# NoemieJaquier/GaBOtorch

Hardware: AMD Instinct MI355X
Metric: SPD affine-invariant kernel-matrix build, pairs/sec (N=4096,d=10) (higher is better)
Workload: dtype f64

## Files before the change

gabotorch_amd/csrc/gabo_mirror.hpp:

```cpp
#pragma once
#include "gabo_device.hpp"

namespace gabo {

template <int TAG>
__global__ __launch_bounds__(256) void mirror_upper_kernel(double* __restrict__ out, int64_t n, int tiles) {
    __shared__ double tile[32][33];
    const int64_t b = blockIdx.y;
    int64_t t = blockIdx.x;
    int ti = 0;
    while (t >= tiles - ti) { t -= tiles - ti; ++ti; }
    int tj = ti + (int)t;
    double* o = out + b * n * n;
    const int tx = threadIdx.x & 31, ty = threadIdx.x >> 5;
    for (int r = ty; r < 32; r += 8) {
        int64_t i = (int64_t)ti * 32 + r, j = (int64_t)tj * 32 + tx;
        tile[r][tx] = (i < n && j < n) ? o[i * n + j] : 0.0;
    }
    __syncthreads();
    for (int r = ty; r < 32; r += 8) {
        int64_t j = (int64_t)tj * 32 + r, i = (int64_t)ti * 32 + tx;
        if (i < n && j < n && i < j) o[j * n + i] = tile[tx][r];
    }
}

__host__ __device__ inline int64_t sym_chunks_of(int64_t cg, int cols, int rows, int64_t row_chunks) {
    int64_t cnt = ((cg + 1) * (int64_t)cols + rows - 1) / rows;
    return cnt < row_chunks ? cnt : row_chunks;
}

__host__ __device__ inline void lower_tile_of(int64_t t, int64_t& bi, int64_t& bj) {
    int64_t r = (int64_t)((__builtin_sqrt(8.0 * (double)t + 1.0) - 1.0) * 0.5);
    while (r * (r + 1) / 2 > t) --r;
    while ((r + 1) * (r + 2) / 2 <= t) ++r;
    bi = r;
    bj = t - r * (r + 1) / 2;
}

}
```

gabotorch_amd/csrc/spd_pairwise_body.hpp:

```cpp
#pragma once
#include "gabo_device.hpp"
#include "spd_eig.hpp"
#include "spd_prep.hpp"
#include "gabo_mirror.hpp"
#include "spd_generic.hpp"
#include "gabo_log_tab.hpp"
#include "gabo_exp_tab256.hpp"
#include "gabo_acosh2_table.hpp"
#include "../../include/gabo_hip.h"

#ifndef GABO_PAIR_WAVES
#define GABO_PAIR_WAVES 2
#else
#define GABO_PAIR_WAVES_FORCED 1
#endif

namespace gabo {

typedef const double __attribute__((address_space(1)))* spd_gcol_ptr;

struct SpdGcolBuffer {
    __amdgpu_buffer_rsrc_t rsrc;
    int voff;
    int stride_bytes;
// ... 31 lines not shown
    constexpr SpdWGroups<D, (GABO_PAIR_WLIM < D ? D : GABO_PAIR_WLIM)> kG{};
    double gq[D][D];
    double wq[2][D][D];
    double c[D];
    auto issue_g = [&](auto ss) {
        constexpr int col = D - 1 - decltype(ss)::value;
        static_for<D - col>([&](auto kk) { gq[col][decltype(kk)::value] = Gj[tri(col + decltype(kk)::value, col)]; });
    };
    auto issue_w = [&](auto gg) {
        constexpr int g = decltype(gg)::value, col = kG.col[g], r0 = kG.r0[g], r1 = kG.r1[g];
        typedef const double __attribute__((address_space(4)))* wrow_ptr;
        wrow_ptr Wg = (wrow_ptr)W;
        asm volatile("" : "+s"(Wg));
        static_for<r1 - r0>([&](auto rr) {
            constexpr int r = r0 + decltype(rr)::value;
            static_for<r - col + 1>([&](auto kk) { wq[g & 1][r][col + decltype(kk)::value] = Wg[tri(r, col + decltype(kk)::value)]; });
        });
    };
    static_for<(AHEAD < D ? AHEAD : D)>(issue_g);
    issue_w(std::integral_constant<int, 0>{});
    static_for<kG.n>([&](auto gg) {
        constexpr int g = decltype(gg)::value, col = kG.col[g], r0 = kG.r0[g], r1 = kG.r1[g];
        if constexpr (r0 == col && D - 1 - col + AHEAD < D) issue_g(std::integral_constant<int, D - 1 - col + AHEAD>{});
        __builtin_amdgcn_sched_barrier(0);
        __builtin_amdgcn_s_waitcnt(0xc07f);
        __builtin_amdgcn_sched_barrier(0);
        if constexpr (g + 1 < kG.n) issue_w(std::integral_constant<int, g + 1>{});
        static_for<r1 - r0>([&](auto rr) {
            constexpr int r = r0 + decltype(rr)::value;
            double acc = wq[g & 1][r][col] * gq[col][0];
            static_for<r - col>([&](auto kk) {
                constexpr int k = col + 1 + decltype(kk)::value;
                acc = __builtin_fma(wq[g & 1][r][k], gq[col][k - col], acc);
            });
            c[r - col] = acc;
        });
        if constexpr (r1 == D) {
            __builtin_amdgcn_sched_barrier(0);
            static_for<D - col>([&](auto rr) {
                constexpr int r = col + decltype(rr)::value;
                static_for<r - col + 1>([&](auto qq) {
                    constexpr int q = col + decltype(qq)::value;
                    m[tri(r, q)] = col == q ? c[r - col] * c[q - col] : __builtin_fma(c[r - col], c[q - col], m[tri(r, q)]);
                });
            });
        }
    });
    __builtin_amdgcn_sched_barrier(0);
}

__constant__ double kLogTabRegs[8] = {1.41421356237309504880, 1.0 / 7.0, -1.0 / 6.0, 0.2, -0.25, 1.0 / 3.0, 6.93147180369123816490e-01,
                                      1.90821492927058770002e-10};
__device__ __forceinline__ LogTabRegs log_tab_regs_scalar() {
    typedef const double __attribute__((address_space(4)))* const_ptr;
    const_ptr p = (const_ptr)kLogTabRegs;
    asm volatile("" : "+s"(p));
    LogTabRegs t;
    t.sqrt2 = p[0], t.c7 = p[1], t.c6 = p[2], t.c5 = p[3], t.c4 = p[4], t.c3 = p[5], t.ln2_hi = p[6], t.ln2_lo = p[7];
    return t;
}

template <int D, int ORIENT = kQlOrientPerLane, int CTL = kQlCtlPlain, int AHEAD = 0, class GCOL>
__device__ __forceinline__ double ai_sumsq(const double* __restrict__ W, const GCOL& Gj, const double* __restrict__ ltab, const double eps2 = 0.0) {
    constexpr int T = tri_size(D);
    constexpr bool kDescending = ORIENT == kQlOrientLast;
    double m[T];
    if constexpr (AHEAD > 0) {
        static_assert(kDescending, "the staged congruence takes the columns from the last to the first");
        ai_congruence_staged<D, AHEAD>(W, Gj, m);
    } else
    static_for<D>([&](auto cc) {
        constexpr int col = kDescending ? D - 1 - decltype(cc)::value : decltype(cc)::value;
        double g[D - col], c[D - col];
        static_for<D - col>([&](auto kk) { g[decltype(kk)::value] = Gj[tri(col + decltype(kk)::value, col)]; });
        static_for<D - col>([&](auto rr) {
            constexpr int r = col + decltype(rr)::value;
            double acc = W[tri(r, col)] * g[0];
            static_for<r - col>([&](auto kk) {
                constexpr int k = col + 1 + decltype(kk)::value;
                acc = __builtin_fma(W[tri(r, k)], g[k - col], acc);
            });
            c[r - col] = acc;
        });
        static_for<D - col>([&](auto rr) {
            constexpr int r = col + decltype(rr)::value;
            static_for<r - col + 1>([&](auto qq) {
                constexpr int q = col + decltype(qq)::value;
                m[tri(r, q)] = (kDescending ? col == q : col == 0) ? c[r - col] * c[q - col] : __builtin_fma(c[r - col], c[q - col], m[tri(r, q)]);
            });
        });
    });
    double dg[D], e2[D];
    tridiagonalize<D, ORIENT>(m, dg, e2);
    tridiag_eigenvalues<D, ORIENT, CTL>(dg, e2, eps2);
    double s = 0.0;
    const LogTabRegs lr = AHEAD > 0 ? log_tab_regs_scalar() : LogTabRegs::load();
    static_for<D>([&](auto kk) { double lg = log_tab(dg[decltype(kk)::value], lr, ltab); s = __builtin_fma(lg, lg, s); });
    return s;
}

struct Spd2Col {
    double g00, g10, g11, lg;
};
__device__ __forceinline__ double ai_sumsq2(const double* __restrict__ W, const Spd2Col& g, double lw, const LogTabRegs& lr,
                                            const double* __restrict__ ltab, double tiny) {
    const double c00 = W[0] * g.g00, c11 = W[2] * g.g11;
    const double c10 = __builtin_fma(W[1], g.g00, W[2] * g.g10);
    const double m00 = c00 * c00, m10d = (c10 + c10) * c00, m11 = __builtin_fma(c10, c10, c11 * c11);
    const double tr = m00 + m11, df = m00 - m11;
    const double root = sqrt_nz(__builtin_fma(df, df, __builtin_fma(m10d, m10d, tiny)));
    const double l1 = log_tab(0.5 * (tr + root), lr, ltab);
    const double l2 = __builtin_fma(2.0, lw + g.lg, -l1);
    return __builtin_fma(l1, l1, l2 * l2);
}

__device__ __forceinline__ double finish(double dist, double beta, int mode) {
    if (mode == GABO_OUT_DISTANCE) return dist;
    if (mode == GABO_OUT_LAPLACE) return exp(-(dist * beta));
    return exp(-((dist * dist) * beta));
}

#ifndef GABO_PAIR_TWO_WAVE_MAX_DIM
#define GABO_PAIR_TWO_WAVE_MAX_DIM 14
#endif
#ifndef GABO_QL_EPS2_GAUSS
#define GABO_QL_EPS2_GAUSS 1e-14
#endif
constexpr bool spd_pair_gauss_only_instantiated(int d) { return d > 2 && d != 12; }
#ifndef GABO_PAIR_ORIENT
constexpr int spd_pair_gauss_only_orientation(int d) { return d == 14 ? kQlOrientCol0 : kQlOrientLast; }
#else
constexpr int spd_pair_gauss_only_orientation(int d) { return GABO_PAIR_ORIENT; }
#endif
#ifndef GABO_PAIR_SWEEPCTL
constexpr int spd_pair_gauss_only_sweepctl(int d) { return d == 20 ? kQlCtlPlain : (kQlCtlDenormalZero | kQlCtlHwSqrt | kQlCtlStageThreshold); }
#else
constexpr int spd_pair_gauss_only_sweepctl(int d) { return GABO_PAIR_SWEEPCTL; }
#endif
#ifndef GABO_PAIR_WAVES_FORCED
constexpr int spd_pair_gauss_only_waves(int d) { return d > GABO_PAIR_TWO_WAVE_MAX_DIM ? 1 : (d == 10 ? 3 : GABO_PAIR_WAVES); }
#else
constexpr int spd_pair_gauss_only_waves(int d) { return d > GABO_PAIR_TWO_WAVE_MAX_DIM ? 1 : GABO_PAIR_WAVES; }
#endif
#ifndef GABO_PAIR_AHEAD
constexpr int spd_pair_gauss_only_ahead(int d) { return d == 10 && spd_pair_gauss_only_waves(d) == 3 ? 2 : 0; }
#else
constexpr int spd_pair_gauss_only_ahead(int d) { return d == 10 ? GABO_PAIR_AHEAD : 0; }
#endif
template <int D, bool GAUSS_ONLY, bool BUFFER_ONLY>
__global__ __launch_bounds__(256, (GAUSS_ONLY ? spd_pair_gauss_only_waves(D) : (D > GABO_PAIR_TWO_WAVE_MAX_DIM ? 1 : GABO_PAIR_WAVES))) void spd_ai_pairwise_kernel(const double* __restrict__ Winv, const double* __restrict__ G,
                                                              double* __restrict__ out, double* __restrict__ dist_out_arg,
                                                              int64_t n1, int64_t n2,
                                                              int64_t w_batch_stride, int64_t g_batch_stride, int rows,
                                                              int col_blocks, int row_chunks, int64_t sym_tiles, double beta, int flags) {
    constexpr int T = tri_size(D);
    static_assert(GAUSS_ONLY == BUFFER_ONLY && (spd_pair_gauss_only_instantiated(D) || !GAUSS_ONLY), "instantiations that launch_spd_ai selects");
    const int mode = GAUSS_ONLY ? GABO_OUT_GAUSSIAN : (flags & GABO_OUT_MASK);
    double* const dist_out = GAUSS_ONLY ? nullptr : dist_out_arg;
    constexpr bool kTabExp = D <= 4;
    __shared__ double tab[kTabExp ? 64 : 1];
    __shared__ __attribute__((aligned(16))) double ltab[512];
    for (int k = threadIdx.x; k < 512; k += blockDim.x) ltab[k] = kLogTab[k];
    double ec[6], ec3 = 0.0;
    if constexpr (kTabExp) {
        if (threadIdx.x < 64) tab[threadIdx.x] = kExp2Tab[threadIdx.x];
    }
    __syncthreads();
    if constexpr (kTabExp) {
        static_for<6>([&](auto k) { ec[decltype(k)::value] = kExpTabC[decltype(k)::value]; });
        ec3 = ec[3];
        asm volatile("" : "+v"(ec3));
    }
    int64_t cg, rc, b;
    if (flags & GABO_SYMMETRIC) {
        const int64_t per_batch = sym_tiles;
        b = blockIdx.x / per_batch;
        int64_t t = blockIdx.x - b * per_batch;
        cg = 0;
        for (;;) {
            int64_t cnt = ((cg + 1) * (int64_t)blockDim.x + rows - 1) / rows;
            if (cnt > row_chunks) cnt = row_chunks;
            if (t < cnt) break;
            t -= cnt;
            ++cg;
        }
        rc = t;
    } else {
        const int64_t bid = blockIdx.x;
        cg = bid % col_blocks;
        rc = (bid / col_blocks) % row_chunks;
        b = bid / ((int64_t)col_blocks * row_chunks);
    }
    const int64_t j0 = cg * blockDim.x;
    const int64_t j = j0 + threadIdx.x;
    const int64_t jc = j < n2 ? j : n2 - 1;
    const int64_t i0 = rc * rows;
    const int64_t i1 = (i0 + rows < n1) ? i0 + rows : n1;
    if ((flags & GABO_SYMMETRIC) && j0 + (int64_t)(threadIdx.x | 63) < i0) return;
    const double* Gj = G + b * g_batch_stride + jc;
    double* ob = out + b * n1 * n2;
    const int64_t jw = j0 + (threadIdx.x & ~63);
    const bool use_buffer = BUFFER_ONLY || (D > 2 && (int64_t)T * n2 * 8 < (1ll << 31));
    SpdGcolBuffer gbuf;
    {
        const double* gw = G + b * g_batch_stride + (jw < n2 ? jw : n2 - 1);
        uint64_t a = (uint64_t)gw;
        a = ((uint64_t)(uint32_t)__builtin_amdgcn_readfirstlane((int)(a >> 32)) << 32) | (uint32_t)__builtin_amdgcn_readfirstlane((int)a);
        gbuf.rsrc = __builtin_amdgcn_make_buffer_rsrc((void*)a, 0, 0x7fffffff, 0x00020000);
        gbuf.voff = (int)((jc - (jw < n2 ? jw : n2 - 1)) * 8);
        gbuf.stride_bytes = (int)(n2 * 8);
    }
    Spd2Col col2;
    double lw_lane = 0.0, tiny = 1e-290;
    LogTabRegs lr2;
    if constexpr (D == 2) {
        lr2 = LogTabRegs::load();
        asm volatile("" : "+s"(tiny));
        col2.g00 = Gj[0];
        col2.g10 = Gj[n2];
        col2.g11 = Gj[2 * n2];
        col2.lg = log_tab(col2.g00 * col2.g11, lr2, ltab);
        int64_t ir = i0 + (threadIdx.x & 63);
        ir = ir < n1 ? ir : n1 - 1;
        const double* Wr = Winv + b * w_batch_stride + ir * T;
        lw_lane = log_tab(Wr[0] * Wr[2], lr2, ltab);
    }
    double eps2 = (mode == GABO_OUT_GAUSSIAN && !dist_out) ? GABO_QL_EPS2_GAUSS : 0.0;
    asm volatile("" : "+s"(eps2));
    if constexpr (GAUSS_ONLY && BUFFER_ONLY) {
        const int nrows = __builtin_amdgcn_readfirstlane((int)(i1 - i0));
        const int64_t jrel = j - i0;
        const int rmax = j >= n2 ? -1 : ((flags & GABO_SYMMETRIC) ? (jrel < 0 ? -1 : (jrel > rows - 1 ? rows - 1 : (int)jrel)) : rows - 1);
        const double* W = Winv + b * w_batch_stride + i0 * T;
        char* orow = reinterpret_cast<char*>(ob + i0 * n2 + j);
        for (int r = 0; r < nrows; ++r, W += T) {
            SpdGcolBuffer gb = gbuf;
            asm volatile("" : "+v"(gb.voff));
            asm volatile("" : "+s"(gb.stride_bytes));
            const double s = ai_sumsq<D, spd_pair_gauss_only_orientation(D), spd_pair_gauss_only_sweepctl(D), spd_pair_gauss_only_ahead(D)>(W, gb, ltab, eps2);
            double val;
            if constexpr (kTabExp) {
                val = exp_neg_tab(-((s + 1e-15) * beta), ec, ec3, tab);
                val = s != s ? s : val;
            } else {
                val = exp(-((s + 1e-15) * beta));
            }
            if (r <= rmax) *reinterpret_cast<double*>(orow) = val;
            orow += (unsigned)gb.stride_bytes;
        }
        return;
    }
    for (int64_t i = i0; i < i1; ++i) {
        const double* W = Winv + b * w_batch_stride + i * T;
        double s;
        if constexpr (D == 2) {
            const int lane = (int)(i - i0);
            const double lw = __hiloint2double(__builtin_amdgcn_readlane(__double2hiint(lw_lane), lane),
                                               __builtin_amdgcn_readlane(__double2loint(lw_lane), lane));
            s = ai_sumsq2(W, col2, lw, lr2, ltab, tiny);
        } else {
            if (use_buffer) {
                SpdGcolBuffer gb = gbuf;
                asm volatile("" : "+v"(gb.voff));
                asm volatile("" : "+s"(gb.stride_bytes));
                s = ai_sumsq<D>(W, gb, ltab, eps2);
            } else {
                SpdGcolPointer gp{(spd_gcol_ptr)Gj, n2};
                asm volatile("" : "+v"(gp.p));
                s = ai_sumsq<D>(W, gp, ltab, eps2);
            }
        }
        double dist, val;
        if (mode == GABO_OUT_GAUSSIAN && !dist_out) {
            dist = 0.0;
            if constexpr (kTabExp) {
                val = exp_neg_tab(-((s + 1e-15) * beta), ec, ec3, tab);
                val = s != s ? s : val;
            } else {
                val = exp(-((s + 1e-15) * beta));
            }
        } else {
            dist = __builtin_sqrt(s + 1e-15);
            val = finish(dist, beta, mode);
        }
        if (j < n2 && (!(flags & GABO_SYMMETRIC) || i <= j)) {
            ob[i * n2 + j] = val;
            if (dist_out) dist_out[b * n1 * n2 + i * n2 + j] = dist;
        }
    }
}

#ifndef GABO_GAUSS2_MAX_ROWS
#define GABO_GAUSS2_MAX_ROWS 64
#endif
constexpr double kGauss2L = 0.0027076061740622863;
__constant__ double kGauss2C[6] = {kGauss2L, kGauss2L * kGauss2L / 2.0, kGauss2L * kGauss2L * kGauss2L / 6.0,
                                   kGauss2L * kGauss2L * kGauss2L * kGauss2L / 24.0, 6755399441055744.0, 4096.0};

template <bool NT, bool SYM>
__global__ __launch_bounds__(256) void spd_ai_gauss2_kernel(const double* __restrict__ Winv, const double* __restrict__ G,
                                                            double* __restrict__ out, int64_t n1, int64_t n2, int64_t w_batch_stride,
                                                            int64_t g_batch_stride, int rows, int col_blocks, int row_chunks,
                                                            int64_t sym_tiles, double beta, int flags) {
    __shared__ __attribute__((aligned(16))) double ltab[512];
    __shared__ double etab[256];
    __shared__ __attribute__((aligned(16))) double atab[kAcosh2Slots * kAcosh2Stride];
    __shared__ __attribute__((aligned(16))) double wrow[GABO_GAUSS2_MAX_ROWS * 4];
    const int tid = threadIdx.x;
    for (int k = tid; k < 512; k += blockDim.x) ltab[k] = kLogTab[k];
    for (int k = tid; k < 256; k += blockDim.x) etab[k] = kExp2Tab256[k];
    {
        const double sc = beta * (-512.0 / 0.69314718055994530942), eps = beta * (-256.0 / 0.69314718055994530942) * 1e-15;
        constexpr int kUsedLo = (kAcosh2Binades - 1) * 16 * kAcosh2Stride, kUsedHi = 240 * kAcosh2Stride;
        for (int k = tid; k < kAcosh2Slots * kAcosh2Stride - (kUsedHi - kUsedLo); k += blockDim.x) {
            const int kk = k < kUsedLo ? k : k + (kUsedHi - kUsedLo);
            const double v = kAcosh2Tab[kk] * sc;
            atab[kk] = (kk % kAcosh2Stride == 0) ? v + eps : v;
        }
    }
    int64_t cg, rc, b;
    if constexpr (SYM) {
        const int64_t per_batch = sym_tiles;
        b = blockIdx.x / per_batch;
        int64_t t = blockIdx.x - b * per_batch;
        cg = 0;
        for (;;) {
            int64_t cnt = ((cg + 1) * (int64_t)blockDim.x + rows - 1) / rows;
            if (cnt > row_chunks) cnt = row_chunks;
            if (t < cnt) break;
            t -= cnt;
            ++cg;
        }
        rc = t;
    } else {
        const int64_t bid = blockIdx.x;
        cg = bid % col_blocks;
        rc = (bid / col_blocks) % row_chunks;
        b = bid / ((int64_t)col_blocks * row_chunks);
    }
    const int64_t j0 = cg * blockDim.x;
    const int64_t j = j0 + tid;
    const int64_t jc = j < n2 ? j : n2 - 1;
    const int64_t i0 = rc * rows;
    const int64_t i1 = (i0 + rows < n1) ? i0 + rows : n1;
    const double* Gj = G + b * g_batch_stride + jc;
    const double g00 = Gj[0], g10 = Gj[n2], g11 = Gj[2 * n2];
    const LogTabRegs lr = LogTabRegs::load();
    const double sscale = __builtin_sqrt(beta * (512.0 / 0.69314718055994530942));
    double w0l = 1.0, w1l = 0.0, w2l = 1.0;
    if (tid < rows) {
        int64_t ir = i0 + tid;
        ir = ir < n1 ? ir : n1 - 1;
        const double* Wr = Winv + b * w_batch_stride + ir * 3;
        w0l = Wr[0], w1l = Wr[1], w2l = Wr[2];
    }
    __syncthreads();
    if (tid < rows) {
        const double dw = w0l * w2l;
        const double sw = rsqrt_nz(dw + dw);
        wrow[4 * tid + 0] = w0l * sw;
        wrow[4 * tid + 1] = w1l * sw;
        wrow[4 * tid + 2] = w2l * sw;
        wrow[4 * tid + 3] = sscale * log_tab(dw, lr, ltab);
    }
    __syncthreads();
    if (SYM && j0 + (int64_t)(tid | 63) < i0) return;
    double ec[6];
    static_for<6>([&](auto k) { ec[decltype(k)::value] = kGauss2C[decltype(k)::value]; });
    double c4v = ec[3];
    asm volatile("" : "+v"(c4v));
    const double dg = g00 * g11;
    const double bcol = sscale * log_tab(dg, lr, ltab);
    const double sg = rsqrt_nz(dg);
    const double q00 = g00 * sg, q10 = g10 * sg, q11 = g11 * sg;
    double* orow = out + b * n1 * n2 + i0 * n2 + j;
    const int nrows = __builtin_amdgcn_readfirstlane((int)(i1 - i0));
    const int64_t jrel = j - i0;
    const int rmax = j >= n2 ? -1 : (SYM ? (jrel < 0 ? -1 : (jrel > GABO_GAUSS2_MAX_ROWS - 1 ? GABO_GAUSS2_MAX_ROWS - 1 : (int)jrel)) : GABO_GAUSS2_MAX_ROWS - 1);
    typedef double g2_v2d __attribute__((ext_vector_type(2)));
    if (!SYM && j >= n2) return;
    for (int r = 0; r < nrows; ++r, orow += n2) {
        const g2_v2d wa = *reinterpret_cast<const g2_v2d*>(wrow + 4 * r);
        const g2_v2d wb = *reinterpret_cast<const g2_v2d*>(wrow + 4 * r + 2);
        const double w0 = wa[0], w1 = wa[1], w2 = wb[0], arow = wb[1];
        const double hh = __builtin_fma(w0, q00, -(w2 * q11));
        const double cc = __builtin_fma(w1, q00, w2 * q10);
        const double tau = __builtin_fma(cc, cc, __builtin_fma(hh, hh, 1.0));
        const unsigned hi = (unsigned)__double2hiint(tau);
        static_assert(kAcosh2MBits == 4 && kAcosh2Slots == 256, "row index = 8 bits");
        const unsigned off = __umul24((hi >> 16) & 0xffu, (unsigned)(kAcosh2Stride * sizeof(double)));
        const double t = tau - __hiloint2double((int)(hi & ~((1u << (20 - kAcosh2MBits)) - 1u)), 0);
        const g2_v2d* row = reinterpret_cast<const g2_v2d*>(reinterpret_cast<const char*>(atab) + off);
        static_assert(kAcosh2Deg == 7, "four coefficient pairs");
        const g2_v2d c67 = row[3], c45 = row[2], c23 = row[1], c01 = row[0];
        double ya = __builtin_fma(c67[1], t, c67[0]);
        ya = __builtin_fma(ya, t, c45[1]);
        ya = __builtin_fma(ya, t, c45[0]);
        ya = __builtin_fma(ya, t, c23[1]);
        ya = __builtin_fma(ya, t, c23[0]);
        ya = __builtin_fma(ya, t, c01[1]);
        ya = __builtin_fma(ya, t, c01[0]);
        if (__builtin_expect(__any(!(tau < ec[5])), 0)) {
            if (!(tau < ec[5])) {
                const double dl = log(tau + __builtin_sqrt(__builtin_fma(tau, tau, -1.0)));
                ya = -(sscale * sscale) * __builtin_fma(dl, dl, 0.5e-15);
            }
        }
        const double sp = arow + bcol;
        const double y = __builtin_fma(-sp, sp, ya);
        const double km = y + ec[4];
        const double kk = km - ec[4];
        const double rr = y - kk;
        double p = __builtin_fma(rr, c4v, ec[2]);
        p = __builtin_fma(p, rr, ec[1]);
        p = __builtin_fma(p, rr, ec[0]);
        p = p * rr;
        const int ki = __double2loint(km);
        const double e = etab[ki & 255];
        const double val = __builtin_ldexp(__builtin_fma(e, p, e), ki >> 8);
        if (!SYM || r <= rmax) {
            if constexpr (NT) __builtin_nontemporal_store(val, orow);
            else *orow = val;
        }
    }
}

template <int D>
static int launch_spd_ai(const double* x1, const double* x2, double* out, double* dist_out, int64_t batch, int64_t n1, int64_t n2,
                         int64_t s1, int64_t s2, double beta, int flags, double* ws, int* status, hipStream_t st, bool prepared = false) {
    constexpr int T = tri_size(D);
    const int64_t b1 = (s1 == 0) ? 1 : batch;
    const int64_t b2 = (s2 == 0) ? 1 : batch;
    double* W = ws;
    double* G = ws + b1 * n1 * T;
    if (!prepared) launch_spd_prep<D>(x1, x2, W, G, b1, b2, n1, n2, s1, s2, status, st, 1);
#ifndef GABO_PAIR_THREADS
#define GABO_PAIR_THREADS (D >= 7 ? 64 : 256)
#endif
    int threads = n2 >= 256 ? GABO_PAIR_THREADS : (n2 > 128 ? 192 : (n2 > 64 ? 128 : 64));
    int64_t col_blocks = (n2 + threads - 1) / threads;
#ifndef GABO_PAIR_ROWS_D2
#define GABO_PAIR_ROWS_D2 16
#endif
#ifndef GABO_PAIR_ROWS
#define GABO_PAIR_ROWS (D >= 9 ? 8 : 16)
#endif
#ifndef GABO_PAIR_ROWS_GAUSS2
#define GABO_PAIR_ROWS_GAUSS2 64
#endif
    const bool gauss2 = D == 2 && (flags & GABO_OUT_MASK) == GABO_OUT_GAUSSIAN && !dist_out && beta >= 0.0;
    int rows = D == 2 ? (gauss2 ? GABO_PAIR_ROWS_GAUSS2 : GABO_PAIR_ROWS_D2) : GABO_PAIR_ROWS;
    while (rows > 1 && col_blocks * ((n1 + rows - 1) / rows) * batch < (rows > 16 ? 1024 : 4096)) rows >>= 1;
    int64_t row_chunks = (n1 + rows - 1) / rows;
    int64_t sym_tiles = 0;
    if (flags & GABO_SYMMETRIC) {
        for (int64_t cg = 0; cg < col_blocks; ++cg) {
            int64_t cnt = ((cg + 1) * threads + rows - 1) / rows;
            sym_tiles += cnt < row_chunks ? cnt : row_chunks;
        }
    }
    int64_t nblocks = ((flags & GABO_SYMMETRIC) ? sym_tiles : col_blocks * row_chunks) * batch;
    if (nblocks > 0x7fffffffLL) return GABO_ERR_ARG;
    bool special2 = false;
    if constexpr (D == 2) special2 = gauss2 && rows <= GABO_GAUSS2_MAX_ROWS;
    if (special2) {
        const bool streaming = batch * n1 * n2 * 8 > (32ll << 20) && !(flags & GABO_SYMMETRIC);
#define GABO_GAUSS2_LAUNCH(...)                                                                                                     \
        hipLaunchKernelGGL((spd_ai_gauss2_kernel<__VA_ARGS__>), dim3((unsigned)nblocks), dim3(threads), 0, st, W, G, out, n1, n2,           \
                           (s1 == 0) ? (int64_t)0 : n1 * T, (s2 == 0) ? (int64_t)0 : n2 * T, rows, (int)col_blocks, (int)row_chunks,       \
                           sym_tiles, beta, flags)
        if (flags & GABO_SYMMETRIC) GABO_GAUSS2_LAUNCH(false, true);
        else if (streaming) GABO_GAUSS2_LAUNCH(true, false);
        else GABO_GAUSS2_LAUNCH(false, false);
#undef GABO_GAUSS2_LAUNCH
    } else {
#define GABO_PAIR_LAUNCH(...)                                                                                                             \
        hipLaunchKernelGGL((spd_ai_pairwise_kernel<D, __VA_ARGS__>), dim3((unsigned)nblocks), dim3(threads), 0, st, W, G, out, dist_out, n1, n2, \
                           (s1 == 0) ? (int64_t)0 : n1 * T, (s2 == 0) ? (int64_t)0 : n2 * T, rows, (int)col_blocks, (int)row_chunks,       \
                           sym_tiles, beta, flags)
        bool gauss_only = false;
        if constexpr (spd_pair_gauss_only_instantiated(D)) {
            gauss_only = (flags & GABO_OUT_MASK) == GABO_OUT_GAUSSIAN && !dist_out && (int64_t)T * n2 * 8 < (1ll << 31);
            if (gauss_only) GABO_PAIR_LAUNCH(true, true);
        }
        if (!gauss_only) GABO_PAIR_LAUNCH(false, false);
#undef GABO_PAIR_LAUNCH
    }
    if (flags & GABO_SYMMETRIC) {
        int tiles = (int)((n1 + 31) / 32);
        hipLaunchKernelGGL((mirror_upper_kernel<0>), dim3((unsigned)((int64_t)tiles * (tiles + 1) / 2), (unsigned)batch), dim3(256), 0, st,
                           out, n1, tiles);
        if (dist_out)
            hipLaunchKernelGGL((mirror_upper_kernel<0>), dim3((unsigned)((int64_t)tiles * (tiles + 1) / 2), (unsigned)batch), dim3(256), 0,
                               st, dist_out, n1, tiles);
    }
    return hipGetLastError() == hipSuccess ? GABO_OK : GABO_ERR_LAUNCH;
}

}

namespace gabo {
int launch_spd_ai_prepared(int d, double* out, int64_t batch, int64_t n1, int64_t n2, bool shared1, bool shared2, double beta, int flags,
                           double* ws, hipStream_t st);
int launch_spd_ai_wide2(int d, const double* x1, const double* x2, double* out, double* dist_out, int64_t batch, int64_t n1, int64_t n2,
                        int64_t s1, int64_t s2, double beta, int flags, double* ws, int* status, hipStream_t st);
int launch_spd_ai_wide3(int d, const double* x1, const double* x2, double* out, double* dist_out, int64_t batch, int64_t n1, int64_t n2,
                        int64_t s1, int64_t s2, double beta, int flags, double* ws, int* status, hipStream_t st);
int launch_spd_ai_wide(int d, const double* x1, const double* x2, double* out, double* dist_out, int64_t batch, int64_t n1, int64_t n2,
                       int64_t s1, int64_t s2, double beta, int flags, double* ws, int* status, hipStream_t st);
}
```

gabotorch_amd/csrc/sphere_pairwise.hip:

```cpp
#include "gabo_device.hpp"
#include "gabo_mirror.hpp"
#include "gabo_exp_tab256.hpp"
#include "gabo_sphere_pw_table.hpp"
#include "gabo_sphere_ktab.hpp"
#include "../../include/gabo_hip.h"

namespace gabo {


constexpr int kSphWDeg = 17;
#define GABO_SPH_P_COEFFS                                                                                                              \
    0.9999999999999998, 0.3333333333336239, 0.17777777771542846, 0.11428571957076086, 0.081269605781923, 0.061574423044727364,         \
    0.048599889486560285, 0.04118585704847234, 0.02076148720348778, 0.11067290731777447, -0.3792345962104177, 1.5080499520508546,      \
    -4.072870215777421, 8.329550989544446, -12.110677571177652, 12.080701723504074, -7.375868506853218, 2.1474532497337413
__constant__ double kSphW[kSphWDeg + 1] = {GABO_SPH_P_COEFFS};
__constant__ double kSphC[8] = {0.010830424695086549 / 4, 1.162596423439437e-12 / 4, 92.33248261689366 * 4, 1.0 / 6.0, 1.0 / 24.0,
                                6755399441055744.0, 3.14159265358979311600e+00, 4.996003610813204e-16};

struct SphPoly {
    double w[kSphWDeg + 1], a, b;
};
static const double kSphWHost[kSphWDeg + 1] = {GABO_SPH_P_COEFFS};

struct SphGauss {
// ... 487 lines not shown
                res = order == 1 ? gv * a : gv * (a * a - 2.0 * beta * (t1 * t1 + th * t2));
            }
            if (!inside) res = 0.0;
        }
        out[g] = res;
    }
}

}

extern "C" int gabo_sphere_from_inner(const double* inner, double* out, int64_t n, double beta, int flags, int order,
                                      gabo_stream_t stream) {
    if (n < 0 || order < 0 || order > 2) return GABO_ERR_ARG;
    if (n == 0) return GABO_OK;
    if (!inner || !out) return GABO_ERR_ARG;
    int64_t blocks = (n + 255) / 256;
    if (blocks > 16384) blocks = 16384;
    hipLaunchKernelGGL(gabo::sphere_from_inner_kernel, dim3((unsigned)blocks), dim3(256), 0, (hipStream_t)stream, inner, out, n, beta,
                       flags & GABO_OUT_MASK, order);
    return hipGetLastError() == hipSuccess ? GABO_OK : GABO_ERR_LAUNCH;
}

namespace gabo {
static bool sphere_uses_ktable(int64_t batch, int64_t n1, int64_t n2, int dim, double beta, int flags) {
    const bool scaled = (flags & GABO_OUT_MASK) == GABO_OUT_GAUSSIAN && beta > 1e-30 && beta < 1000.0;
    return scaled && beta <= kSphKtMaxBeta && dim <= 16 && n2 >= 1024 && (double)batch * (double)n1 * (double)n2 >= (double)(1 << 22);
}

__global__ __launch_bounds__(256) void sphere_ktable_kernel(double beta, double* __restrict__ table) {
    const int s = blockIdx.x * blockDim.x + threadIdx.x;
    if (s < kSphKtSlots) sphere_kt_build_row(s, SphKtBaseRow::load(s), beta, table);
}
}

extern "C" int64_t gabo_sphere_ktable_doubles(void) { return (int64_t)gabo::kSphKtSlots * gabo::kSphKtStride; }

extern "C" int gabo_sphere_pairwise_uses_ktable(int64_t batch, int64_t n1, int64_t n2, int dim, double beta, int flags, int diag) {
    return (!diag && gabo::sphere_uses_ktable(batch, n1, n2, dim, beta, flags)) ? 1 : 0;
}

extern "C" int gabo_sphere_ktable_build(double beta, double* table, gabo_stream_t stream) {
    if (!table || !(beta > 1e-30) || beta > gabo::kSphKtMaxBeta) return GABO_ERR_ARG;
    hipLaunchKernelGGL(gabo::sphere_ktable_kernel, dim3((gabo::kSphKtSlots + 255) / 256), dim3(256), 0, (hipStream_t)stream, beta, table);
    return hipGetLastError() == hipSuccess ? GABO_OK : GABO_ERR_LAUNCH;
}

extern "C" int gabo_sphere_pairwise_cached(const double* x1, const double* x2, double* out, int64_t batch, int64_t n1, int64_t n2,
                                           int dim, int64_t x1_batch_stride, int64_t x2_batch_stride, double beta, int flags,
                                           int diag, const double* ktable, gabo_stream_t stream);

extern "C" int gabo_sphere_pairwise(const double* x1, const double* x2, double* out, int64_t batch, int64_t n1, int64_t n2,
                                    int dim, int64_t x1_batch_stride, int64_t x2_batch_stride, double beta, int flags,
                                    int diag, gabo_stream_t stream) {
    return gabo_sphere_pairwise_cached(x1, x2, out, batch, n1, n2, dim, x1_batch_stride, x2_batch_stride, beta, flags, diag, nullptr, stream);
}

extern "C" int gabo_sphere_pairwise_cached(const double* x1, const double* x2, double* out, int64_t batch, int64_t n1, int64_t n2,
                                           int dim, int64_t x1_batch_stride, int64_t x2_batch_stride, double beta, int flags,
                                           int diag, const double* ktable, gabo_stream_t stream) {
    if (batch < 0 || n1 < 0 || n2 < 0 || x1_batch_stride < 0 || x2_batch_stride < 0) return GABO_ERR_ARG;
    if (dim < 1) return GABO_ERR_DIM;
    if (batch == 0 || n1 == 0 || n2 == 0) return GABO_OK;
    if (!x1 || !x2 || !out) return GABO_ERR_ARG;
    hipStream_t st = (hipStream_t)stream;
    if (diag) {
        if (n1 != n2) return GABO_ERR_ARG;
        int64_t tot = batch * n1;
        hipLaunchKernelGGL(gabo::sphere_diag_kernel, dim3((unsigned)((tot + 255) / 256)), dim3(256), 0, st, x1, x2, out, batch, n1,
                           dim, x1_batch_stride, x2_batch_stride, beta, flags);
    } else {
        if (batch > 65535) return GABO_ERR_ARG;
        const int mode = flags & GABO_OUT_MASK;
        const bool scaled = mode == GABO_OUT_GAUSSIAN && beta > 1e-30 && beta < 1000.0;
        const bool kt = gabo::sphere_uses_ktable(batch, n1, n2, dim, beta, flags);
#ifndef GABO_SPH_KT_THREADS
#define GABO_SPH_KT_THREADS ((((n2 + 1023) / 1024) * ((n1 + 16 * gabo::kSphKtChunks - 1) / (16 * gabo::kSphKtChunks)) * batch <= 320) ? 1024 : 512)
#endif
        const int kt_threads = GABO_SPH_KT_THREADS;
        int threads = kt ? kt_threads : (n2 >= 256 ? 256 : (n2 > 128 ? 192 : (n2 > 64 ? 128 : 64)));
        int64_t col_blocks = (n2 + threads - 1) / threads;
#ifndef GABO_SPH_CHUNKS
#define GABO_SPH_CHUNKS 4
#endif
        static_assert(GABO_SPH_CHUNKS <= gabo::kSphMaxChunks, "LDS copy of the x1 rows");
        int chunks = kt ? gabo::kSphKtChunks : GABO_SPH_CHUNKS;
        while (chunks > 1 && col_blocks * ((n1 + 16 * chunks - 1) / (16 * chunks)) * batch < (kt ? 256 * (1024 / kt_threads) : 1024)) chunks >>= 1;
        const int rows = 16 * chunks;
        int64_t row_chunks = (n1 + rows - 1) / rows;
        int64_t tiles_x = col_blocks * row_chunks;
        if (flags & GABO_SYMMETRIC) {
            if (n1 != n2) return GABO_ERR_ARG;
            tiles_x = 0;
            for (int64_t cg = 0; cg < col_blocks; ++cg) tiles_x += gabo::sym_chunks_of(cg, threads, rows, row_chunks);
        }
        if (tiles_x > 0x7fffffffLL) return GABO_ERR_ARG;
        gabo::SphPoly poly = {};
        if (scaled) {
            const double sc = 4.0 * beta, pi = 3.14159265358979311600e+00;
            for (int k = 0; k <= gabo::kSphWDeg; ++k) poly.w[k] = gabo::kSphWHost[k] * sc;
            poly.a = 2.0 * pi * sqrt(beta);
            poly.b = beta * (pi * pi);
        }
#ifndef GABO_SPH_NT_BYTES
#define GABO_SPH_NT_BYTES (32ll << 20)
#endif
        const bool streaming = batch * n1 * n2 * 8 > GABO_SPH_NT_BYTES && !(flags & GABO_SYMMETRIC);
#define GABO_SPH_LAUNCH_NT(M, SC, K, NT_)                                                                                          \
    hipLaunchKernelGGL((gabo::sphere_pairwise_kernel<M, SC, K, NT_, SC>), dim3((unsigned)tiles_x, (unsigned)batch),                    \
                       dim3(threads), 0, st, x1, x2, out, n1, n2, dim, x1_batch_stride, x2_batch_stride, (int)col_blocks, (int)row_chunks, \
                       chunks, beta, flags, poly, (const double*)nullptr)
#define GABO_SPH_LAUNCH_KT(K, NT_)                                                                                                 \
    hipLaunchKernelGGL((gabo::sphere_pairwise_kernel<GABO_OUT_GAUSSIAN, true, K, NT_, false, true>), dim3((unsigned)tiles_x, (unsigned)batch), \
                       dim3(threads), 0, st, x1, x2, out, n1, n2, dim, x1_batch_stride, x2_batch_stride, (int)col_blocks, (int)row_chunks, \
                       chunks, beta, flags, poly, ktable)
#ifndef GABO_SPH_KT_NT
#define GABO_SPH_KT_NT 0
#endif
#define GABO_SPH_LAUNCH_KT_KS(K)                                                                                                   \
    do {                                                                                                                           \
        if (streaming && GABO_SPH_KT_NT) GABO_SPH_LAUNCH_KT(K, (GABO_SPH_KT_NT != 0));                                             \
        else GABO_SPH_LAUNCH_KT(K, false);                                                                                         \
    } while (0)
#define GABO_SPH_LAUNCH_KS(M, SC, K)                                                                                               \
    do {                                                                                                                           \
        if (streaming) GABO_SPH_LAUNCH_NT(M, SC, K, true);                                                                         \
        else GABO_SPH_LAUNCH_NT(M, SC, K, false);                                                                                  \
    } while (0)
#define GABO_SPH_LAUNCH(M, SC)                                                                                                     \
    do {                                                                                                                           \
        switch (dim <= 16 ? (dim + 3) / 4 : 0) {                                                                                   \
            case 1: GABO_SPH_LAUNCH_KS(M, SC, 1); break;                                                                           \
            case 2: GABO_SPH_LAUNCH_KS(M, SC, 2); break;                                                                           \
            case 3: GABO_SPH_LAUNCH_KS(M, SC, 3); break;                                                                           \
            case 4: GABO_SPH_LAUNCH_KS(M, SC, 4); break;                                                                           \
            default: GABO_SPH_LAUNCH_KS(M, SC, 0); break;                                                                          \
        }                                                                                                                          \
    } while (0)
        if (kt) {
            switch ((dim + 3) / 4) {
                case 1: GABO_SPH_LAUNCH_KT_KS(1); break;
                case 2: GABO_SPH_LAUNCH_KT_KS(2); break;
                case 3: GABO_SPH_LAUNCH_KT_KS(3); break;
                default: GABO_SPH_LAUNCH_KT_KS(4); break;
            }
        } else if (mode == GABO_OUT_DISTANCE) GABO_SPH_LAUNCH(GABO_OUT_DISTANCE, false);
        else if (mode == GABO_OUT_LAPLACE) GABO_SPH_LAUNCH(GABO_OUT_LAPLACE, false);
        else if (scaled) GABO_SPH_LAUNCH(GABO_OUT_GAUSSIAN, true);
        else GABO_SPH_LAUNCH(GABO_OUT_GAUSSIAN, false);
#undef GABO_SPH_LAUNCH
#undef GABO_SPH_LAUNCH_KS
#undef GABO_SPH_LAUNCH_NT
#undef GABO_SPH_LAUNCH_KT_KS
#undef GABO_SPH_LAUNCH_KT
        if (flags & GABO_SYMMETRIC) {
            int tiles = (int)((n1 + 31) / 32);
            hipLaunchKernelGGL((gabo::mirror_upper_kernel<1>), dim3((unsigned)((int64_t)tiles * (tiles + 1) / 2), (unsigned)batch),
                               dim3(256), 0, st, out, n1, tiles);
        }
    }
    return hipGetLastError() == hipSuccess ? GABO_OK : GABO_ERR_LAUNCH;
}
```

gabotorch_amd/csrc/sphere_zonal.hip:

```cpp
#include "gabo_device.hpp"
#include "gabo_mirror.hpp"
#include "sphere_zonal_level.hpp"
#include "../../include/gabo_hip.h"

namespace gabo {

struct ZonalSeries {
    ZonalLevel lv[kZonalMaxCoeff + 3];
    int n;
};

template <int NV>
__device__ __forceinline__ void zonal_eval(const ZonalSeries& s, const double (&c)[NV], double (&f)[NV]) {
    double p0[NV], p1[NV];
    const double a0 = s.lv[0].a, a1 = s.lv[1].a;
    static_for<NV>([&](auto vv) {
        constexpr int v = decltype(vv)::value;
        p0[v] = 1.0;
        p1[v] = c[v];
        f[v] = __builtin_fma(a1, c[v], a0);
    });
    const int n = s.n;
    ZonalLevel e = s.lv[2], o = s.lv[3];
    int k = 2;
// ... 20 lines not shown
        });
    }
}

__global__ __launch_bounds__(256) void sphere_zonal_from_inner_kernel(const double* __restrict__ cin, double* __restrict__ out, int64_t n,
                                                                      const ZonalSeries s) {
    const int64_t T = (int64_t)gridDim.x * blockDim.x;
    for (int64_t base = (int64_t)blockIdx.x * blockDim.x + threadIdx.x; base < n; base += 4 * T) {
        double c[4], f[4];
        static_for<4>([&](auto vv) {
            const int64_t g = base + decltype(vv)::value * T;
            c[decltype(vv)::value] = cin[g < n ? g : n - 1];
        });
        zonal_eval<4>(s, c, f);
        static_for<4>([&](auto vv) {
            const int64_t g = base + decltype(vv)::value * T;
            if (g < n) out[g] = f[decltype(vv)::value];
        });
    }
}

typedef double zon_v4d __attribute__((ext_vector_type(4)));

__global__ __launch_bounds__(256) void sphere_zonal_pairwise_kernel(const double* __restrict__ x1, const double* __restrict__ x2,
                                                                    double* __restrict__ out, int64_t n1, int64_t n2, int dim, int64_t s1,
                                                                    int64_t s2, int col_blocks, int chunks, int flags, const ZonalSeries s) {
    const int tid = threadIdx.x;
    const uint32_t rc = blockIdx.x / (uint32_t)col_blocks, cg = blockIdx.x - rc * (uint32_t)col_blocks;
    const int64_t b = blockIdx.y;
    const int lane = tid & 63, li = lane & 15, lk = lane >> 4;
    const int64_t j0 = (int64_t)cg * blockDim.x + 64 * __builtin_amdgcn_readfirstlane(tid >> 6);
    if (j0 >= n2) return;
    const bool sym = (flags & GABO_SYMMETRIC) != 0;
    const double* pb[4];
    static_for<4>([&](auto tt) {
        constexpr int t = decltype(tt)::value;
        int64_t jb = j0 + 16 * t + li;
        jb = jb < n2 ? jb : n2 - 1;
        pb[t] = x2 + b * s2 + jb * dim;
    });
    double* ob = out + b * n1 * n2;
    for (int ch = 0; ch < chunks; ++ch) {
        const int64_t i0 = ((int64_t)rc * chunks + ch) * 16;
        if (i0 >= n1) break;
        if (sym && j0 + 63 < i0) break;
        const int64_t ia = (i0 + li < n1) ? i0 + li : n1 - 1;
        const double* pa = x1 + b * s1 + ia * dim;
        zon_v4d acc[4];
        auto kstep = [&](int k0, auto first) {
            const int kk = k0 + lk;
            const bool ok = kk < dim;
            const int kc = ok ? kk : dim - 1;
            double a = pa[kc];
            double bv[4];
            static_for<4>([&](auto tt) { bv[decltype(tt)::value] = pb[decltype(tt)::value][kc]; });
            a = ok ? a : 0.0;
            static_for<4>([&](auto tt) { bv[decltype(tt)::value] = ok ? bv[decltype(tt)::value] : 0.0; });
            static_for<4>([&](auto tt) {
                constexpr int t = decltype(tt)::value;
                if constexpr (decltype(first)::value) acc[t] = __builtin_amdgcn_mfma_f64_16x16x4f64(a, bv[t], zon_v4d{0.0, 0.0, 0.0, 0.0}, 0, 0, 0);
                else acc[t] = __builtin_amdgcn_mfma_f64_16x16x4f64(a, bv[t], acc[t], 0, 0, 0);
            });
        };
        kstep(0, std::true_type{});
        for (int k0 = 4; k0 < dim; k0 += 4) kstep(k0, std::false_type{});
        static_for<2>([&](auto hh) {
            constexpr int T0 = 2 * decltype(hh)::value;
            double c[8], f[8];
            static_for<8>([&](auto ee) { c[decltype(ee)::value] = acc[T0 + (decltype(ee)::value >> 2)][decltype(ee)::value & 3]; });
            zonal_eval<8>(s, c, f);
            static_for<2>([&](auto tt) {
                constexpr int t = T0 + decltype(tt)::value;
                const int64_t j = j0 + 16 * t + li;
                static_for<4>([&](auto rr) {
                    constexpr int r = decltype(rr)::value;
                    const int64_t i = i0 + lk + 4 * r;
                    if (i < n1 && j < n2 && (!sym || i <= j)) ob[i * n2 + j] = f[4 * decltype(tt)::value + r];
                });
            });
            __builtin_amdgcn_sched_barrier(0);
        });
    }
}

__global__ __launch_bounds__(256) void sphere_zonal_diag_kernel(const double* __restrict__ x1, const double* __restrict__ x2,
                                                                double* __restrict__ out, int64_t batch, int64_t n, int dim, int64_t s1,
                                                                int64_t s2, const ZonalSeries s) {
    const int64_t g = (int64_t)blockIdx.x * blockDim.x + threadIdx.x;
    if (g >= batch * n) return;
    const int64_t b = g / n, i = g - b * n;
    const double* p = x1 + b * s1 + i * dim;
    const double* q = x2 + b * s2 + i * dim;
    double c[1] = {0.0}, f[1];
    for (int k = 0; k < dim; ++k) c[0] = __builtin_fma(p[k], q[k], c[0]);
    zonal_eval<1>(s, c, f);
    out[g] = f[0];
}

static int zonal_series(const double* coeff_host, int n_coeff, int series_dim, ZonalSeries& s) {
    if (n_coeff < 1 || n_coeff > kZonalMaxCoeff || !coeff_host) return GABO_ERR_ARG;
    if (series_dim < 1) return GABO_ERR_DIM;
    s = ZonalSeries{};
    s.n = n_coeff;
    for (int k = 0; k < n_coeff; ++k) {
        s.lv[k].a = coeff_host[k];
        if (k >= 2) s.lv[k].rb = ((double)k - 1.0) / ((double)k + (double)series_dim - 2.0);
    }
    return GABO_OK;
}

}

extern "C" int gabo_sphere_zonal_from_inner(const double* inner, double* out, int64_t n, const double* coeff_host, int n_coeff,
                                            int series_dim, gabo_stream_t stream) {
    gabo::ZonalSeries s;
    const int rc = gabo::zonal_series(coeff_host, n_coeff, series_dim, s);
    if (rc != GABO_OK) return rc;
    if (n < 0) return GABO_ERR_ARG;
    if (n == 0) return GABO_OK;
    if (!inner || !out) return GABO_ERR_ARG;
    int64_t blocks = (n + 1023) / 1024;
    if (blocks > 16384) blocks = 16384;
    hipLaunchKernelGGL(gabo::sphere_zonal_from_inner_kernel, dim3((unsigned)blocks), dim3(256), 0, (hipStream_t)stream, inner, out, n, s);
    return hipGetLastError() == hipSuccess ? GABO_OK : GABO_ERR_LAUNCH;
}

extern "C" int gabo_sphere_zonal_pairwise(const double* x1, const double* x2, double* out, int64_t batch, int64_t n1, int64_t n2, int dim,
                                          int64_t x1_batch_stride, int64_t x2_batch_stride, const double* coeff_host, int n_coeff,
                                          int series_dim, int flags, int diag, gabo_stream_t stream) {
    gabo::ZonalSeries s;
    const int rcs = gabo::zonal_series(coeff_host, n_coeff, series_dim, s);
    if (rcs != GABO_OK) return rcs;
    if (batch < 0 || n1 < 0 || n2 < 0 || x1_batch_stride < 0 || x2_batch_stride < 0) return GABO_ERR_ARG;
    if (dim < 1) return GABO_ERR_DIM;
    if (diag ? n1 != n2 : (batch > 65535 || ((flags & GABO_SYMMETRIC) && n1 != n2))) return GABO_ERR_ARG;
    if (batch == 0 || n1 == 0 || n2 == 0) return GABO_OK;
    if (!x1 || !x2 || !out) return GABO_ERR_ARG;
    hipStream_t st = (hipStream_t)stream;
    if (diag) {
        const int64_t tot = batch * n1;
        if ((tot + 255) / 256 > 0x7fffffffLL) return GABO_ERR_ARG;
        hipLaunchKernelGGL(gabo::sphere_zonal_diag_kernel, dim3((unsigned)((tot + 255) / 256)), dim3(256), 0, st, x1, x2, out, batch, n1, dim,
                           x1_batch_stride, x2_batch_stride, s);
    } else {
        const int threads = n2 >= 256 ? 256 : (n2 > 128 ? 192 : (n2 > 64 ? 128 : 64));
        const int64_t col_blocks = (n2 + threads - 1) / threads;
        int chunks = 4;
        while (chunks > 1 && col_blocks * ((n1 + 16 * chunks - 1) / (16 * chunks)) * batch < 1024) chunks >>= 1;
        const int64_t row_chunks = (n1 + 16 * chunks - 1) / (16 * chunks);
        const int64_t tiles_x = col_blocks * row_chunks;
        if (tiles_x > 0x7fffffffLL) return GABO_ERR_ARG;
        hipLaunchKernelGGL(gabo::sphere_zonal_pairwise_kernel, dim3((unsigned)tiles_x, (unsigned)batch), dim3(threads), 0, st, x1, x2, out, n1,
                           n2, dim, x1_batch_stride, x2_batch_stride, (int)col_blocks, chunks, flags, s);
        if (flags & GABO_SYMMETRIC) {
            const int tiles = (int)((n1 + 31) / 32);
            hipLaunchKernelGGL((gabo::mirror_upper_kernel<5>), dim3((unsigned)((int64_t)tiles * (tiles + 1) / 2), (unsigned)batch), dim3(256), 0,
                               st, out, n1, tiles);
        }
    }
    return hipGetLastError() == hipSuccess ? GABO_OK : GABO_ERR_LAUNCH;
}
```

Baseline: 8.289 billion.

## Rework symmetric tile indexing, mirror kernel tiling, and symmetric row chunking

Replaces the linear-scan symmetric tile decode with a closed-form sqrt-based mapping and puts the batch index in blockIdx.y. The upper-to-lower mirror kernel now uses 64x64 tiles with optional 2-wide vector loads and stores, launches tiles in reverse order, and skips loading the lower half of diagonal tiles. For D>=9 the symmetric path uses 4 rows per block, giving finer triangular granularity and less wasted work above the diagonal. These aim to cut per-block decode overhead, mirror bandwidth cost and triangle waste, at the cost of more blocks and a new batch limit of 65535.

```diff
diff --git a/gabotorch_amd/csrc/gabo_mirror.hpp b/gabotorch_amd/csrc/gabo_mirror.hpp
--- a/gabotorch_amd/csrc/gabo_mirror.hpp
+++ b/gabotorch_amd/csrc/gabo_mirror.hpp
@@ -2,27 +2,6 @@
 #include "gabo_device.hpp"
 
 namespace gabo {
-
-template <int TAG>
-__global__ __launch_bounds__(256) void mirror_upper_kernel(double* __restrict__ out, int64_t n, int tiles) {
-    __shared__ double tile[32][33];
-    const int64_t b = blockIdx.y;
-    int64_t t = blockIdx.x;
-    int ti = 0;
-    while (t >= tiles - ti) { t -= tiles - ti; ++ti; }
-    int tj = ti + (int)t;
-    double* o = out + b * n * n;
-    const int tx = threadIdx.x & 31, ty = threadIdx.x >> 5;
-    for (int r = ty; r < 32; r += 8) {
-        int64_t i = (int64_t)ti * 32 + r, j = (int64_t)tj * 32 + tx;
-        tile[r][tx] = (i < n && j < n) ? o[i * n + j] : 0.0;
-    }
-    __syncthreads();
-    for (int r = ty; r < 32; r += 8) {
-        int64_t j = (int64_t)tj * 32 + r, i = (int64_t)ti * 32 + tx;
-        if (i < n && j < n && i < j) o[j * n + i] = tile[tx][r];
-    }
-}
 
 __host__ __device__ inline int64_t sym_chunks_of(int64_t cg, int cols, int rows, int64_t row_chunks) {
     int64_t cnt = ((cg + 1) * (int64_t)cols + rows - 1) / rows;
@@ -37,4 +16,68 @@
     bj = t - r * (r + 1) / 2;
 }
 
+__host__ __device__ inline void sym_tile_of(int64_t t, int q, int col_blocks, int64_t& cg, int64_t& rc) {
+    int64_t c = (int64_t)((__builtin_sqrt(8.0 * (double)t / (double)q + 1.0) - 1.0) * 0.5);
+    while (c > 0 && ((q * c * (c + 1)) >> 1) > t) --c;
+    while (((q * (c + 1) * (c + 2)) >> 1) <= t) ++c;
+    if (c > col_blocks - 1) c = col_blocks - 1;
+    cg = c;
+    rc = t - ((q * c * (c + 1)) >> 1);
 }
+
+constexpr int kMirrorTile = 64;
+template <int TAG, int VEC>
+__global__ __launch_bounds__(256) void mirror_upper_kernel(double* __restrict__ out, int64_t n, int tiles) {
+    static_assert(VEC == 1 || VEC == 2, "doubles per access");
+    constexpr int TS = kMirrorTile, LANES = TS / VEC, STEP = 256 / LANES;
+    typedef double vec_t __attribute__((ext_vector_type(VEC)));
+    __shared__ double tile[TS][TS + 1];
+    int64_t tj64, ti64;
+    lower_tile_of((int64_t)gridDim.x - 1 - blockIdx.x, tj64, ti64);
+    if (tj64 > tiles - 1) return;
+    const int64_t i0 = ti64 * TS, j0 = tj64 * TS;
+    const bool diagonal = ti64 == tj64;
+    double* o = out + (int64_t)blockIdx.y * n * n;
+    const int tx = (threadIdx.x % LANES) * VEC, ty = threadIdx.x / LANES;
+    for (int r = ty; r < TS; r += STEP) {
+        const int64_t i = i0 + r, j = j0 + tx;
+        if (i < n && j < n && (!diagonal || tx + VEC - 1 > r)) {
+            if constexpr (VEC == 2) {
+                const vec_t v = *reinterpret_cast<const vec_t*>(o + i * n + j);
+                tile[r][tx] = v[0];
+                tile[r][tx + 1] = v[1];
+            } else {
+                tile[r][tx] = o[i * n + j];
+            }
+        }
+    }
+    __syncthreads();
+    for (int r = ty; r < TS; r += STEP) {
+        const int64_t j = j0 + r, i = i0 + tx;
+        if (j >= n || i >= n || i >= j) continue;
+        if constexpr (VEC == 2) {
+            if (i + 1 < j) {
+                vec_t v;
+                v[0] = tile[tx][r];
+                v[1] = tile[tx + 1][r];
+                *reinterpret_cast<vec_t*>(o + j * n + i) = v;
+            } else {
+                o[j * n + i] = tile[tx][r];
+            }
+        } else {
+            o[j * n + i] = tile[tx][r];
+        }
+    }
+}
+
+template <int TAG>
+static void launch_mirror_upper(double* out, int64_t n, int64_t batch, hipStream_t st) {
+    const int tiles = (int)((n + kMirrorTile - 1) / kMirrorTile);
+    const dim3 grid((unsigned)((int64_t)tiles * (tiles + 1) / 2), (unsigned)batch);
+    if (n % 2 == 0 && reinterpret_cast<uintptr_t>(out) % 16 == 0)
+        hipLaunchKernelGGL((mirror_upper_kernel<TAG, 2>), grid, dim3(256), 0, st, out, n, tiles);
+    else
+        hipLaunchKernelGGL((mirror_upper_kernel<TAG, 1>), grid, dim3(256), 0, st, out, n, tiles);
+}
+
+}
diff --git a/gabotorch_amd/csrc/spd_pairwise_body.hpp b/gabotorch_amd/csrc/spd_pairwise_body.hpp
--- a/gabotorch_amd/csrc/spd_pairwise_body.hpp
+++ b/gabotorch_amd/csrc/spd_pairwise_body.hpp
@@ -207,7 +207,7 @@
                                                               double* __restrict__ out, double* __restrict__ dist_out_arg,
                                                               int64_t n1, int64_t n2,
                                                               int64_t w_batch_stride, int64_t g_batch_stride, int rows,
-                                                              int col_blocks, int row_chunks, int64_t sym_tiles, double beta, int flags) {
+                                                              int col_blocks, int row_chunks, int sym_q, double beta, int flags) {
     constexpr int T = tri_size(D);
     static_assert(GAUSS_ONLY == BUFFER_ONLY && (spd_pair_gauss_only_instantiated(D) || !GAUSS_ONLY), "instantiations that launch_spd_ai selects");
     const int mode = GAUSS_ONLY ? GABO_OUT_GAUSSIAN : (flags & GABO_OUT_MASK);
@@ -228,18 +228,8 @@
     }
     int64_t cg, rc, b;
     if (flags & GABO_SYMMETRIC) {
-        const int64_t per_batch = sym_tiles;
-        b = blockIdx.x / per_batch;
-        int64_t t = blockIdx.x - b * per_batch;
-        cg = 0;
-        for (;;) {
-            int64_t cnt = ((cg + 1) * (int64_t)blockDim.x + rows - 1) / rows;
-            if (cnt > row_chunks) cnt = row_chunks;
-            if (t < cnt) break;
-            t -= cnt;
-            ++cg;
-        }
-        rc = t;
+        b = blockIdx.y;
+        sym_tile_of((int64_t)blockIdx.x, sym_q, col_blocks, cg, rc);
     } else {
         const int64_t bid = blockIdx.x;
         cg = bid % col_blocks;
@@ -356,7 +346,7 @@
 __global__ __launch_bounds__(256) void spd_ai_gauss2_kernel(const double* __restrict__ Winv, const double* __restrict__ G,
                                                             double* __restrict__ out, int64_t n1, int64_t n2, int64_t w_batch_stride,
                                                             int64_t g_batch_stride, int rows, int col_blocks, int row_chunks,
-                                                            int64_t sym_tiles, double beta, int flags) {
+                                                            int sym_q, double beta, int flags) {
     __shared__ __attribute__((aligned(16))) double ltab[512];
     __shared__ double etab[256];
     __shared__ __attribute__((aligned(16))) double atab[kAcosh2Slots * kAcosh2Stride];
@@ -375,18 +365,8 @@
     }
     int64_t cg, rc, b;
     if constexpr (SYM) {
-        const int64_t per_batch = sym_tiles;
-        b = blockIdx.x / per_batch;
-        int64_t t = blockIdx.x - b * per_batch;
-        cg = 0;
-        for (;;) {
-            int64_t cnt = ((cg + 1) * (int64_t)blockDim.x + rows - 1) / rows;
-            if (cnt > row_chunks) cnt = row_chunks;
-            if (t < cnt) break;
-            t -= cnt;
-            ++cg;
-        }
-        rc = t;
+        b = blockIdx.y;
+        sym_tile_of((int64_t)blockIdx.x, sym_q, col_blocks, cg, rc);
     } else {
         const int64_t bid = blockIdx.x;
         cg = bid % col_blocks;
@@ -504,35 +484,40 @@
 #define GABO_PAIR_ROWS_GAUSS2 64
 #endif
     const bool gauss2 = D == 2 && (flags & GABO_OUT_MASK) == GABO_OUT_GAUSSIAN && !dist_out && beta >= 0.0;
-    int rows = D == 2 ? (gauss2 ? GABO_PAIR_ROWS_GAUSS2 : GABO_PAIR_ROWS_D2) : GABO_PAIR_ROWS;
+#ifndef GABO_PAIR_ROWS_SYM
+#define GABO_PAIR_ROWS_SYM (D >= 9 ? 4 : GABO_PAIR_ROWS)
+#endif
+    int rows = D == 2 ? (gauss2 ? GABO_PAIR_ROWS_GAUSS2 : GABO_PAIR_ROWS_D2) : ((flags & GABO_SYMMETRIC) ? GABO_PAIR_ROWS_SYM : GABO_PAIR_ROWS);
     while (rows > 1 && col_blocks * ((n1 + rows - 1) / rows) * batch < (rows > 16 ? 1024 : 4096)) rows >>= 1;
     int64_t row_chunks = (n1 + rows - 1) / rows;
+    static_assert(64 % (GABO_PAIR_ROWS) == 0 && 64 % (GABO_PAIR_ROWS_SYM) == 0 && 64 % (GABO_PAIR_ROWS_D2) == 0 && 64 % (GABO_PAIR_ROWS_GAUSS2) == 0,
+                  "rows per block: a power of two up to 64");
     int64_t sym_tiles = 0;
     if (flags & GABO_SYMMETRIC) {
-        for (int64_t cg = 0; cg < col_blocks; ++cg) {
-            int64_t cnt = ((cg + 1) * threads + rows - 1) / rows;
-            sym_tiles += cnt < row_chunks ? cnt : row_chunks;
-        }
-    }
-    int64_t nblocks = ((flags & GABO_SYMMETRIC) ? sym_tiles : col_blocks * row_chunks) * batch;
+        if (batch > 65535) return GABO_ERR_ARG;
+        for (int64_t cg = 0; cg < col_blocks; ++cg) sym_tiles += sym_chunks_of(cg, threads, rows, row_chunks);
+    }
+    const int sym_q = threads / rows;
+    int64_t nblocks = (flags & GABO_SYMMETRIC) ? sym_tiles : col_blocks * row_chunks * batch;
     if (nblocks > 0x7fffffffLL) return GABO_ERR_ARG;
+    const dim3 grid((unsigned)nblocks, (flags & GABO_SYMMETRIC) ? (unsigned)batch : 1u);
     bool special2 = false;
     if constexpr (D == 2) special2 = gauss2 && rows <= GABO_GAUSS2_MAX_ROWS;
     if (special2) {
         const bool streaming = batch * n1 * n2 * 8 > (32ll << 20) && !(flags & GABO_SYMMETRIC);
 #define GABO_GAUSS2_LAUNCH(...)                                                                                                     \
-        hipLaunchKernelGGL((spd_ai_gauss2_kernel<__VA_ARGS__>), dim3((unsigned)nblocks), dim3(threads), 0, st, W, G, out, n1, n2,           \
+        hipLaunchKernelGGL((spd_ai_gauss2_kernel<__VA_ARGS__>), grid, dim3(threads), 0, st, W, G, out, n1, n2,                              \
                            (s1 == 0) ? (int64_t)0 : n1 * T, (s2 == 0) ? (int64_t)0 : n2 * T, rows, (int)col_blocks, (int)row_chunks,       \
-                           sym_tiles, beta, flags)
+                           sym_q, beta, flags)
         if (flags & GABO_SYMMETRIC) GABO_GAUSS2_LAUNCH(false, true);
         else if (streaming) GABO_GAUSS2_LAUNCH(true, false);
         else GABO_GAUSS2_LAUNCH(false, false);
 #undef GABO_GAUSS2_LAUNCH
     } else {
 #define GABO_PAIR_LAUNCH(...)                                                                                                             \
-        hipLaunchKernelGGL((spd_ai_pairwise_kernel<D, __VA_ARGS__>), dim3((unsigned)nblocks), dim3(threads), 0, st, W, G, out, dist_out, n1, n2, \
+        hipLaunchKernelGGL((spd_ai_pairwise_kernel<D, __VA_ARGS__>), grid, dim3(threads), 0, st, W, G, out, dist_out, n1, n2,                   \
                            (s1 == 0) ? (int64_t)0 : n1 * T, (s2 == 0) ? (int64_t)0 : n2 * T, rows, (int)col_blocks, (int)row_chunks,       \
-                           sym_tiles, beta, flags)
+                           sym_q, beta, flags)
         bool gauss_only = false;
         if constexpr (spd_pair_gauss_only_instantiated(D)) {
             gauss_only = (flags & GABO_OUT_MASK) == GABO_OUT_GAUSSIAN && !dist_out && (int64_t)T * n2 * 8 < (1ll << 31);
@@ -542,12 +527,8 @@
 #undef GABO_PAIR_LAUNCH
     }
     if (flags & GABO_SYMMETRIC) {
-        int tiles = (int)((n1 + 31) / 32);
-        hipLaunchKernelGGL((mirror_upper_kernel<0>), dim3((unsigned)((int64_t)tiles * (tiles + 1) / 2), (unsigned)batch), dim3(256), 0, st,
-                           out, n1, tiles);
-        if (dist_out)
-            hipLaunchKernelGGL((mirror_upper_kernel<0>), dim3((unsigned)((int64_t)tiles * (tiles + 1) / 2), (unsigned)batch), dim3(256), 0,
-                               st, dist_out, n1, tiles);
+        launch_mirror_upper<0>(out, n1, batch, st);
+        if (dist_out) launch_mirror_upper<0>(dist_out, n1, batch, st);
     }
     return hipGetLastError() == hipSuccess ? GABO_OK : GABO_ERR_LAUNCH;
 }
diff --git a/gabotorch_amd/csrc/sphere_pairwise.hip b/gabotorch_amd/csrc/sphere_pairwise.hip
--- a/gabotorch_amd/csrc/sphere_pairwise.hip
+++ b/gabotorch_amd/csrc/sphere_pairwise.hip
@@ -663,11 +663,7 @@
 #undef GABO_SPH_LAUNCH_NT
 #undef GABO_SPH_LAUNCH_KT_KS
 #undef GABO_SPH_LAUNCH_KT
-        if (flags & GABO_SYMMETRIC) {
-            int tiles = (int)((n1 + 31) / 32);
-            hipLaunchKernelGGL((gabo::mirror_upper_kernel<1>), dim3((unsigned)((int64_t)tiles * (tiles + 1) / 2), (unsigned)batch),
-                               dim3(256), 0, st, out, n1, tiles);
-        }
+        if (flags & GABO_SYMMETRIC) gabo::launch_mirror_upper<1>(out, n1, batch, st);
     }
     return hipGetLastError() == hipSuccess ? GABO_OK : GABO_ERR_LAUNCH;
 }
diff --git a/gabotorch_amd/csrc/sphere_zonal.hip b/gabotorch_amd/csrc/sphere_zonal.hip
--- a/gabotorch_amd/csrc/sphere_zonal.hip
+++ b/gabotorch_amd/csrc/sphere_zonal.hip
@@ -196,11 +196,7 @@
         if (tiles_x > 0x7fffffffLL) return GABO_ERR_ARG;
         hipLaunchKernelGGL(gabo::sphere_zonal_pairwise_kernel, dim3((unsigned)tiles_x, (unsigned)batch), dim3(threads), 0, st, x1, x2, out, n1,
                            n2, dim, x1_batch_stride, x2_batch_stride, (int)col_blocks, chunks, flags, s);
-        if (flags & GABO_SYMMETRIC) {
-            const int tiles = (int)((n1 + 31) / 32);
-            hipLaunchKernelGGL((gabo::mirror_upper_kernel<5>), dim3((unsigned)((int64_t)tiles * (tiles + 1) / 2), (unsigned)batch), dim3(256), 0,
-                               st, out, n1, tiles);
-        }
+        if (flags & GABO_SYMMETRIC) gabo::launch_mirror_upper<5>(out, n1, batch, st);
     }
     return hipGetLastError() == hipSuccess ? GABO_OK : GABO_ERR_LAUNCH;
 }
```

Result: no change. 8.285 billion (-0.0%).
